# interaction-lab-uh/STROTSS-tensorflow

Measured on AMD Instinct MI355X. Metric: optimisation_steps_per_sec_1024px_pair, higher is better.
Workload: dtype f32; 1 GPU; 1024px content/style pair, 1024x1024 scale of the coarse-to-fine pyramid, 1024 samples x D=2179, VGG16 (seeded He-normal weights), RMSprop pixel update; scale_px=1024, samples=1024, parallelism=single GPU, tap_adjoint=deterministic (planned, sorted scatter)

## Files before the change

strotss-tensorflow_amd/csrc/gemm.hip:

```cpp
#include <stdlib.h>

#include "internal.h"
#include "mfma_pipe.h"
#include "mfma_x3.h"

namespace {

template <int BM, int BN, bool AKC, bool BKC>
__device__ __forceinline__ void gemm_mainloop(const float* __restrict__ A, int lda, int M,
                                              const float* __restrict__ B, int ldb, int N, int K,
                                              int m0, int n0, float* ldsA, float* ldsB,
                                              f32x16 (&acc)[BM / 64][BN / 64]) {
  f32x4 ra[BM / 32], rb[BN / 32];
  auto load = [&](int k0) {
    if constexpr (AKC) gload_kc<BM>(ra, A, lda, m0, M, k0); else gload_rc<BM>(ra, A, lda, m0, M, k0);
    if constexpr (BKC) gload_kc<BN>(rb, B, ldb, n0, N, k0); else gload_rc<BN>(rb, B, ldb, n0, N, k0);
  };
  load(0);
  for (int k0 = 0; k0 < K; k0 += 32) {
    __syncthreads();
    if constexpr (AKC) lds_store_kc<BM>(ldsA, ra); else lds_store_rc<BM>(ldsA, ra);
    if constexpr (BKC) lds_store_kc<BN>(ldsB, rb); else lds_store_rc<BN>(ldsB, rb);
    __syncthreads();
    if (k0 + 32 < K) load(k0 + 32);
// ... 340 lines not shown
  const size_t total = (size_t)rows * (K >> 2);
  hipLaunchKernelGGL(x3_split_rows_kernel, dim3((unsigned)min((size_t)2048, (total + 255) / 256), batch), dim3(256), 0, s,
                     x, rows, ld, K, stride_in, (__bf16*)panels, (long long)3 * rows * K);
  ST_LAUNCH_RET();
}

struct EpiScaleStoreX3 : EpiScaleStore, X3NoPrefetch<EpiScaleStoreX3> {
  using EpiScaleStore::apply;
  using X3NoPrefetch<EpiScaleStoreX3>::apply;
};
struct X3NoMirror {
  template <class Epi, class Pre, class Acc, class Map>
  __device__ __forceinline__ void operator()(const Epi&, Pre&, float*, int, int, int, int, Acc&, const Map&) const {}
};
template <class Cfg>
struct X3Mirror {
  template <class Epi, class Pre, class Acc, class Map>
  __device__ __forceinline__ void operator()(const Epi& epi, Pre&, float* tile, int m0, int n0, int M, int N, Acc& acc,
                                             const Map& map) const {
    mirror_tile<Cfg::BM, Cfg::BN, Cfg::NT, true>(epi, tile, m0, n0, M, N, [&](auto put) {
#pragma unroll
      for (int im = 0; im < Cfg::T; ++im)
#pragma unroll
        for (int in = 0; in < Cfg::T; ++in)
#pragma unroll
          for (int reg = 0; reg < 16; ++reg) {
            const int r = m0 + map.row(im, reg), c = n0 + map.colof(in);
            put(r, c, (r < M && c < N) ? epi.value(r, c, acc[im][in][reg]) : 0.f);
          }
    });
  }
};

int st_gemm_x3_batched(const void* A, const void* B, float* C, int ldc, long long strideC, int M, int N, int K,
                       int batch, hipStream_t s, long min_tiles128) {
  EpiScaleStoreX3 e{{C, ldc, M, N, 1.0f, strideC}, {}};
  static const bool k16 = [] { const char* v = getenv("STROTSS_X3_K16"); return !v || atoi(v) != 0; }();
  if ((long)cdiv(N, 128) * cdiv(M, 128) * batch >= min_tiles128 && k16) {
    using Cfg = X3CfgK16<3>;
    dim3 grid((unsigned)cdiv(N, 128) * cdiv(M, 128) * batch);
    hipLaunchKernelGGL((gemm_x3_kernel<Cfg, EpiScaleStoreX3, X3NoMirror>), grid, dim3(Cfg::NT), 0, s, (const __bf16*)A, M,
                       (long long)3 * M * K, (const __bf16*)B, N, (long long)3 * N * K, K, e, X3NoMirror{});
  } else if ((long)cdiv(N, 128) * cdiv(M, 128) * batch >= min_tiles128) {
    using Cfg = X3Cfg<128>;
    dim3 grid((unsigned)cdiv(N, 128) * cdiv(M, 128) * batch);
    hipLaunchKernelGGL((gemm_x3_kernel<Cfg, EpiScaleStoreX3, X3NoMirror>), grid, dim3(Cfg::NT), 0, s, (const __bf16*)A, M,
                       (long long)3 * M * K, (const __bf16*)B, N, (long long)3 * N * K, K, e, X3NoMirror{});
  } else {
    using Cfg = X3Cfg<64>;
    dim3 grid((unsigned)cdiv(N, 64) * cdiv(M, 64) * batch);
    hipLaunchKernelGGL((gemm_x3_kernel<Cfg, EpiScaleStoreX3, X3NoMirror>), grid, dim3(Cfg::NT), 0, s, (const __bf16*)A, M,
                       (long long)3 * M * K, (const __bf16*)B, N, (long long)3 * N * K, K, e, X3NoMirror{});
  }
  ST_LAUNCH_RET();
}

struct EpiSelfsimBwdX3 : EpiSelfsimBwd {
  template <int T> struct Pre { float dx0[T][T][16], x0[T][T][16], ri[T][16], qi[T][16]; };
  template <class P> __device__ __forceinline__ void prefetch(P& p, int im, int in, int reg, int row, int c) const {
    const int rr = min(row, M - 1);
    const size_t o = (size_t)rr * ld + min(c, N - 1);
    p.dx0[im][in][reg] = dx[o];
    p.x0[im][in][reg] = x[o];
    if (in == 0) { p.ri[im][reg] = r[rr]; p.qi[im][reg] = q[rr]; }
  }
  template <class P> __device__ __forceinline__ float apply(P& p, int im, int in, int reg, int row, int c, float v) const {
    const float ri = p.ri[im][reg];
    const float out = p.dx0[im][in][reg] + g * ri * (v - p.x0[im][in][reg] * ri * p.qi[im][reg]);
    if (row < M && c < N) dx[(size_t)row * ld + c] = out;
    return 0.f;
  }
};
struct EpiAxpbyBiasX3 : EpiAxpbyBias {
  template <int T> struct Pre { float c0[T][T][16], b[T]; };
  template <class P> __device__ __forceinline__ void prefetch(P& p, int im, int in, int reg, int r, int c) const {
    p.c0[im][in][reg] = C[(size_t)min(r, M - 1) * ldc + min(c, N - 1)];
    if (im == 0 && reg == 0) p.b[in] = bias[min(c, N - 1)];
  }
  template <class P> __device__ __forceinline__ float apply(P& p, int im, int in, int reg, int r, int c, float v) const {
    const float out = p.c0[im][in][reg] + alpha * v + bias_scale * p.b[in];
    if (r < M && c < N) C[(size_t)r * ldc + c] = out;
    return 0.f;
  }
};
struct EpiMomentFwdX3 {
  static constexpr bool SYMM = true;
// ... 238 lines not shown
```

strotss-tensorflow_amd/csrc/internal.h:

```cpp
#pragma once
#include "common.h"

int st_cosine_distance(const float* x, const float* rx, int nx, const float* y, const float* ry, int ny,
                       int ld, float* C, int ldc, hipStream_t s);
int st_l2_distance(const float* x, const float* xs, int nx, const float* y, const float* ys, int ny, int ld, int d,
                   float* C, int ldc, hipStream_t s);
int st_remd_cost(const float* x, const float* rx, const float* sx, int nx, const float* y, const float* ry, const float* sy,
                 int ny, int ld, int d, int metric, float* C, float* S, int ldc, hipStream_t s);
int st_gram_tn(const float* A, int krows, int ld, float alpha, float* C, hipStream_t s);
int st_moment_fwd_gemm(const float* cy, int krows, int ld, const float* Sx, float* T, float inv_n,
                       float* partial, int* n_partial, hipStream_t s);
int st_moment_bwd_gemm(const float* cy, int n, int ld, const float* T, float alpha, const float* bias,
                       float bias_scale, float* dY, hipStream_t s);
int st_selfsim_bwd_gemm(const float* Mq, int ldm, int kpad, const float* bmat, const float* x, const float* r,
                        const float* q, int n, int ld, float g, float* dx, hipStream_t s);

int st_gemm_nt_batched(const float* A, int lda, long long strideA, const float* B, int ldb, long long strideB,
                       float* C, int ldc, long long strideC, int M, int N, int K, int batch, hipStream_t s);

bool st_winograd43_fused_enabled(int h, int w, int cout);
int st_winograd43_pack(const float* u_prk, int rows, int k, float* u_packed, hipStream_t st);
int st_winograd43_fused(const float* in, int h, int w, int cin, const float* U, const float* bias, int cout,
                        const float* mask, int relu, float* out, float* pool_out, unsigned char* pool_code,
                        const unsigned* bits_in, unsigned* bits_out, hipStream_t st, int accumulate = 0);
int st_maxpool2_fwd(const float* in, int h, int w, int c, float* out, unsigned char* code, hipStream_t st);

int st_x3_split_rows(const float* x, int rows, int ld, int K, long long stride_in, void* panels, int batch,
                     hipStream_t s);
int st_cosine_distance_x3(const void* xp, const float* rx, int nx, const void* yp, const float* ry, int ny, int K,
                          int symm, float* C, int ldc, int batch, long long pstride, long long rstride,
                          long long cstride, hipStream_t s);
int st_selfsim_bwd_x3(const void* Mp, int kpad, const void* Xt, const float* x, const float* r, const float* q, int n,
                      int ld, float g, float* dx, hipStream_t s);
int st_gram_tn_x3(const void* Pt, int npad, int ld, float alpha, float* C, hipStream_t s);
int st_moment_fwd_x3(const void* Pt, int npad, int ld, const float* Sx, void* Tp, float inv_n, float* partial,
                     int* n_partial, hipStream_t s);
int st_loss_forward_group_x3(const void* Pt, int npad, int ld, const float* Sx, void* Tp, float inv_n, float* partial,
                             int* n_partial, const void* xp, const float* rp, int n, long long pstride, long long rstride,
                             float* Dx, int ldc, long long dstride, const void* xs, const float* rs, int ns, float* Ct,
                             int ldt, hipStream_t s);
int st_loss_forward_blend_x3(const void* Pt, int npad, int ld, float inv_n, float* Sigma, const void* xp, const float* rp,
                             int n, long long pstride, long long rstride, float* Dx, int ldc, long long dstride, int n_styles,
                             const void* const* xs, const float* const* rs, const int* ns, float* const* Ct, const int* ldt,
                             hipStream_t s);
int st_moment_bwd_x3_full(const void* Pc, int n, int ld, const void* Sp, float alpha, const float* bias, float bias_scale,
                          float* dY, hipStream_t s);
int st_moment_bwd_x3(const void* Pc, int n, int ld, const void* Tp, float alpha, const float* bias, float bias_scale,
                     float* dY, hipStream_t s);
int st_gemm_x3_batched(const void* A, const void* B, float* C, int ldc, long long strideC, int M, int N, int K,
                       int batch, hipStream_t s, long min_tiles128 = 0);

static inline int round_up(int v, int m) { return (v + m - 1) / m * m; }

struct Workspace {
  char* base; size_t size; size_t off;
  Workspace(void* p, size_t n) : base((char*)p), size(n), off(0) {}
  template <class T> T* take(size_t count) {
    size_t bytes = (count * sizeof(T) + 255) & ~(size_t)255;
    if (off + bytes > size) { failed = true; return nullptr; }
    T* r = reinterpret_cast<T*>(base + off);
    off += bytes;
    return r;
  }
  bool failed = false;
  bool ok() const { return !failed; }
  static Workspace planner() { return Workspace(nullptr, (size_t)1 << 60); }
};
static inline size_t ws_slice(size_t count, size_t elt) { return (count * elt + 255) & ~(size_t)255; }
```

strotss-tensorflow_amd/csrc/mfma_x3.h:

```cpp
#pragma once
#include <type_traits>

#include "mfma_pipe.h"

typedef __bf16 bf16x8 __attribute__((ext_vector_type(8)));
typedef __bf16 bf16x4 __attribute__((ext_vector_type(4)));
typedef unsigned int u32x4 __attribute__((ext_vector_type(4)));

struct Split3 { bf16x4 h, m, l; };
__device__ __forceinline__ Split3 split3(const f32x4 x) {
  Split3 s;
#pragma unroll
  for (int k = 0; k < 4; ++k) {
    const __bf16 h = (__bf16)x[k];
    const float r1 = x[k] - (float)h;
    const __bf16 m = (__bf16)r1;
    const float r2 = r1 - (float)m;
    s.h[k] = h; s.m[k] = m; s.l[k] = (__bf16)r2;
  }
  return s;
}

__host__ __device__ __forceinline__ size_t x3_panel_elems(size_t rows, size_t K) { return 3 * rows * K; }
__device__ __forceinline__ void x3_store4(__bf16* base, size_t rows, size_t row, int k0, const f32x4 v) {
  const Split3 s = split3(v);
  const size_t o = ((size_t)(k0 >> 5) * 3 * rows + row) * 32 + (k0 & 31);
  *reinterpret_cast<bf16x4*>(base + o) = s.h;
  *reinterpret_cast<bf16x4*>(base + o + rows * 32) = s.m;
  *reinterpret_cast<bf16x4*>(base + o + 2 * rows * 32) = s.l;
}

template <int B_, int NPB_ = 3>
struct X3Cfg {
  static_assert(B_ == 128 || B_ == 64, "x3 main loop: 128 x 128 or 64 x 64 tiles");
  static_assert(NPB_ == 3 || (NPB_ == 1 && B_ == 128), "single-plane B: 128 x 128 tiles only");
  static constexpr int NPB = NPB_, NPROD = NPB_ == 3 ? 6 : 3;
  static constexpr int BM = B_, BN = B_, WM = 2, WN = 2, NT = 256;
  static constexpr int T = B_ / 64;
  static constexpr int TM = T, TN = T;
  static constexpr int PL = B_ * 64;
  static constexpr int STAGE = (3 + NPB_) * PL;
  static constexpr int LDS_BYTES = 3 * STAGE;
  static constexpr int G = B_ / 64;
  static constexpr int NP = (3 + NPB_) * G;
  static constexpr bool K16 = false;
};

#define X3_WAIT_VM(n) asm volatile("s_waitcnt vmcnt(" #n ")" ::: "memory")

template <int G, int NPL = 3>
struct X3Operand {
  const char* base;
  unsigned off[G];
  unsigned plane;
  unsigned cur;
  __device__ __forceinline__ X3Operand(const __bf16* p, int rows, int row0) {
    const int lane = threadIdx.x & 63, wave = __builtin_amdgcn_readfirstlane(threadIdx.x >> 6);
    base = reinterpret_cast<const char*>(p);
    plane = (unsigned)rows * 64u;
    cur = 0;
    const int chunk = (lane & 3) ^ ((lane >> 4) & 3);
#pragma unroll
    for (int g = 0; g < G; ++g) {
      const int row = min(row0 + (G * wave + g) * 16 + (lane >> 2), rows - 1);
      off[g] = (unsigned)row * 64u + (unsigned)chunk * 16u;
    }
  }
  __device__ __forceinline__ void dma(int pl, int g, unsigned char* lds_dst) const {
    const char* src = base + (size_t)(cur + pl * plane) + off[g];
    __builtin_amdgcn_global_load_lds((const __attribute__((address_space(1))) void*)src,
                                     (__attribute__((address_space(3))) void*)lds_dst, 16, 0, 0);
  }
  __device__ __forceinline__ void advance() { cur += NPL * plane; }
};

template <class Cfg>
__device__ __forceinline__ void x3_mainloop(unsigned char* lds, int steps, X3Operand<Cfg::G, 3>& oa,
                                            X3Operand<Cfg::G, Cfg::NPB>& ob, f32x16 (&acc)[Cfg::T][Cfg::T]) {
// ... 69 lines not shown
#else
            acc[im][in_][0] += (float)fa[c][PA[q]][im][0] + (float)fb[c][PB[q]][in_][0];
#endif
            const int done = (q * T + im) * T + in_ + 1;
            if (MODE == 2 && c == 0 && done % STRIDE == 0 && done / STRIDE <= NP) {
              __builtin_amdgcn_sched_barrier(0);
              dma_piece(done / STRIDE - 1, s_nn);
              __builtin_amdgcn_sched_barrier(0);
            }
          }
        }
        if (c == 1 && q == 0 && MODE != 0) {
          __builtin_amdgcn_sched_barrier(0);
          if (MODE == 2) wait_one_tile_in_flight(); else X3_WAIT_VM(0);
          asm volatile("s_waitcnt lgkmcnt(0)" ::: "memory");
#ifndef X3_ABL_NO_BARRIER
          __builtin_amdgcn_s_barrier();
#endif
          asm volatile("" ::: "memory");
          read_frags(s_nxt, 0, 0);
          __builtin_amdgcn_sched_barrier(0);
        }
      }
    }
    if (MODE == 2) { oa.advance(); ob.advance(); }
    unsigned char* tmp = s_cur; s_cur = s_nxt; s_nxt = s_nn; s_nn = tmp;
  };
  int s = 0;
  for (; s + 2 < steps; ++s) kstep(std::integral_constant<int, 2>{});
  if (steps > 1) kstep(std::integral_constant<int, 1>{});
  kstep(std::integral_constant<int, 0>{});
}

template <int NPB_ = 3>
struct X3CfgK16 {
  static_assert(NPB_ == 3, "K16 ring: three B planes");
  static constexpr int NPB = NPB_, NPROD = 6;
  static constexpr int BM = 128, BN = 128, WM = 2, WN = 2, NT = 256;
  static constexpr int T = 2, TM = 2, TN = 2;
  static constexpr int PL = 128 * 32;
  static constexpr int STAGE = 6 * PL;
  static constexpr int LDS_BYTES = 3 * STAGE;
  static constexpr int G = 1, NP = 6;
  static constexpr bool K16 = true;
};

struct X3OperandK16 {
  const char* base;
  unsigned off;
  unsigned plane;
  unsigned cur;
  __device__ __forceinline__ X3OperandK16(const __bf16* p, int rows, int row0) {
    const int lane = threadIdx.x & 63, wave = __builtin_amdgcn_readfirstlane(threadIdx.x >> 6);
    base = reinterpret_cast<const char*>(p);
    plane = (unsigned)rows * 64u;
    cur = 0;
    const int row = min(row0 + wave * 32 + (lane >> 1), rows - 1);
    off = (unsigned)row * 64u + (unsigned)((lane & 1) ^ ((lane >> 4) & 1)) * 16u;
  }
  __device__ __forceinline__ void dma(int pl, unsigned char* lds_dst) const {
    const char* src = base + (size_t)(cur + pl * plane) + off;
    __builtin_amdgcn_global_load_lds((const __attribute__((address_space(1))) void*)src,
                                     (__attribute__((address_space(3))) void*)lds_dst, 16, 0, 0);
  }
  __device__ __forceinline__ void advance(int half) { cur += half ? 3u * plane - 32u : 32u; }
};

template <class Cfg> struct X3Ops {
  using A = std::conditional_t<Cfg::K16, X3OperandK16, X3Operand<Cfg::G, 3>>;
  using B = std::conditional_t<Cfg::K16, X3OperandK16, X3Operand<Cfg::G, Cfg::NPB>>;
};

template <class Cfg>
__device__ __forceinline__ void x3_k16_prologue(unsigned char* lds, X3OperandK16& oa, X3OperandK16& ob) {
#ifndef X3_ABL_NO_DMA
  const int wave = __builtin_amdgcn_readfirstlane(threadIdx.x >> 6);
#pragma unroll
  for (int h = 0; h < 2; ++h) {
    unsigned char* stage = lds + h * Cfg::STAGE;
#pragma unroll
    for (int j = 0; j < 6; ++j) {
      unsigned char* dst = stage + j * Cfg::PL + wave * 1024;
      if (j < 3) oa.dma(j, dst); else ob.dma(j - 3, dst);
    }
    oa.advance(h); ob.advance(h);
  }
#endif
}

template <class Cfg>
__device__ __forceinline__ void x3_mainloop_k16(unsigned char* lds, int steps, X3OperandK16& oa, X3OperandK16& ob,
                                                f32x16 (&acc)[2][2]) {
  constexpr int PL = Cfg::PL, STAGE = Cfg::STAGE;
  const int t = threadIdx.x, lane = t & 63, wave = __builtin_amdgcn_readfirstlane(t >> 6);
  const int wm = wave >> 1, wn = wave & 1, l31 = lane & 31, hh = lane >> 5;
  auto dma_piece = [&](int j, unsigned char* stage) {
#ifdef X3_ABL_NO_DMA
    return;
#endif
    unsigned char* dst = stage + j * PL + wave * 1024;
    if (j < 3) oa.dma(j, dst); else ob.dma(j - 3, dst);
  };
  int half = 0;
  const int sw = (hh ^ ((l31 >> 3) & 1)) << 4;
  const int a_rd = (wm * 64 + l31) * 32 + sw;
  const int b_rd = 3 * PL + (wn * 64 + l31) * 32 + sw;
  bf16x8 fa[2][3][2], fb[2][3][2];
  auto read_frags = [&](const unsigned char* stage, int slot) {
#ifdef X3_ABL_NO_FRAG
    if (stage != lds) return;
#endif
#pragma unroll
    for (int p = 0; p < 3; ++p) {
#pragma unroll
      for (int i = 0; i < 2; ++i) {
        fa[slot][p][i] = *reinterpret_cast<const bf16x8*>(stage + a_rd + p * PL + i * 1024);
        fb[slot][p][i] = *reinterpret_cast<const bf16x8*>(stage + b_rd + p * PL + i * 1024);
      }
    }
  };
  constexpr int PA[6] = {2, 0, 1, 1, 0, 0};
  constexpr int PB[6] = {0, 2, 1, 0, 1, 0};

  unsigned char* s_cur = lds;
  unsigned char* s_nxt = lds + STAGE;
  unsigned char* s_nn = lds + 2 * STAGE;
  X3_WAIT_VM(6);
  __builtin_amdgcn_s_barrier();
  read_frags(s_cur, 0);

  auto kstep = [&](auto mode_tag, auto slot_tag) {
    constexpr int MODE = decltype(mode_tag)::value, SLOT = decltype(slot_tag)::value;
#pragma unroll
    for (int q = 0; q < 6; ++q) {
#pragma unroll
      for (int im = 0; im < 2; ++im) {
#pragma unroll
        for (int in_ = 0; in_ < 2; ++in_) {
#ifndef X3_ABL_NO_MFMA
          acc[im][in_] = __builtin_amdgcn_mfma_f32_32x32x16_bf16(fa[SLOT][PA[q]][im], fb[SLOT][PB[q]][in_], acc[im][in_], 0, 0, 0);
#else
          acc[im][in_][0] += (float)fa[SLOT][PA[q]][im][0] + (float)fb[SLOT][PB[q]][in_][0];
#endif
          const int done = (q * 2 + im) * 2 + in_ + 1;
          if (MODE == 2 && done <= 6) {
            __builtin_amdgcn_sched_barrier(0);
            dma_piece(done - 1, s_nn);
            __builtin_amdgcn_sched_barrier(0);
          }
        }
      }
      if (q == 3 && MODE != 0) {
        __builtin_amdgcn_sched_barrier(0);
        if (MODE == 2) X3_WAIT_VM(6); else X3_WAIT_VM(0);
        asm volatile("s_waitcnt lgkmcnt(0)" ::: "memory");
#ifndef X3_ABL_NO_BARRIER
        __builtin_amdgcn_s_barrier();
#endif
        asm volatile("" ::: "memory");
        read_frags(s_nxt, SLOT ^ 1);
        __builtin_amdgcn_sched_barrier(0);
      }
    }
    if (MODE == 2) { oa.advance(half); ob.advance(half); half ^= 1; }
    unsigned char* tmp = s_cur; s_cur = s_nxt; s_nxt = s_nn; s_nn = tmp;
  };
  using I0 = std::integral_constant<int, 0>; using I1 = std::integral_constant<int, 1>; using I2 = std::integral_constant<int, 2>;
  int s = 0;
  for (; s + 3 < steps; s += 2) { kstep(I2{}, I0{}); kstep(I2{}, I1{}); }
  kstep(I1{}, I0{});
  kstep(I0{}, I1{});
}

template <class D>
struct X3NoPrefetch {
  template <int T> struct Pre {};
  template <class P> __device__ __forceinline__ void prefetch(P&, int, int, int, int, int) const {}
  template <class P> __device__ __forceinline__ float apply(P&, int, int, int, int r, int c, float v) const {
    return static_cast<const D*>(this)->apply(r, c, v);
  }
};

template <class Cfg, class Epi, class Mirror>
__device__ __forceinline__ void gemm_x3_tile(unsigned char* lds, unsigned bid, unsigned nblk, const __bf16* __restrict__ A, int M,
                                             long long strideA, const __bf16* __restrict__ B, int N, long long strideB, int K,
                                             const Epi& epi_in, const Mirror& mirror, int xbh, int xbw) {
  Epi epi = epi_in;
  const unsigned gx = (N + Cfg::BN - 1) / Cfg::BN, gy = (M + Cfg::BM - 1) / Cfg::BM;
  unsigned tile = xcd_swizzle(bid, nblk);
  unsigned bz = 0;
  int m0, n0;
  bool tri = false;
  if constexpr (Epi::SYMM) tri = epi.symm != 0;
  if (tri) {
    const unsigned ntri = gx * (gx + 1) / 2;
    bz = tile / ntri;
    tile -= bz * ntri;
    unsigned i = 0, len = gx;
    while (tile >= len) { tile -= len; --len; ++i; }
    m0 = i * Cfg::BM; n0 = (i + tile) * Cfg::BN;
  } else {
    bz = tile / (gx * gy);
    const unsigned rem = tile - bz * (gx * gy);
    if (xbh > 0) {
      const unsigned per = (unsigned)(xbh * xbw), blk = rem / per, in = rem - blk * per;
      const unsigned bpr = gx / (unsigned)xbw;
      const unsigned ty = (blk / bpr) * xbh + in / xbw, tx = (blk % bpr) * xbw + in % xbw;
      m0 = ty * Cfg::BM; n0 = tx * Cfg::BN;
    } else {
      m0 = (rem / gx) * Cfg::BM; n0 = (rem % gx) * Cfg::BN;
    }
  }
  epi.set_batch(bz);
  typename X3Ops<Cfg>::A oa(A + (long long)bz * strideA, M, m0);
  typename X3Ops<Cfg>::B ob(B + (long long)bz * strideB, N, n0);
  f32x16 acc[Cfg::T][Cfg::T];
#pragma unroll
  for (int i = 0; i < Cfg::T; ++i)
#pragma unroll
    for (int j = 0; j < Cfg::T; ++j)
#pragma unroll
      for (int r = 0; r < 16; ++r) acc[i][j][r] = 0.f;
  PipeAccMap<Cfg> map;
  typename Epi::template Pre<Cfg::T> pre;
#pragma unroll
  for (int im = 0; im < Cfg::T; ++im)
#pragma unroll
    for (int in = 0; in < Cfg::T; ++in)
#pragma unroll
      for (int reg = 0; reg < 16; ++reg)
        epi.prefetch(pre, im, in, reg, m0 + map.row(im, reg), n0 + map.colof(in));
  if constexpr (Cfg::K16) { x3_k16_prologue<Cfg>(lds, oa, ob); x3_mainloop_k16<Cfg>(lds, K >> 4, oa, ob, acc); }
  else x3_mainloop<Cfg>(lds, K >> 5, oa, ob, acc);
  float local = 0.f;
#pragma unroll
  for (int im = 0; im < Cfg::T; ++im)
#pragma unroll
    for (int in = 0; in < Cfg::T; ++in)
#pragma unroll
      for (int reg = 0; reg < 16; ++reg)
        local += epi.apply(pre, im, in, reg, m0 + map.row(im, reg), n0 + map.colof(in), acc[im][in][reg]);
  if constexpr (Epi::SYMM) {
    static_assert(!Epi::SYMM || Cfg::LDS_BYTES >= Cfg::BM * (Cfg::BN + 1) * 4, "mirror tile");
    if (epi.symm && n0 >= m0) mirror(epi, pre, reinterpret_cast<float*>(lds), m0, n0, M, N, acc, map);
  }
  __syncthreads();
  epi.finish(reinterpret_cast<float*>(lds), local);
}

template <class Cfg, class Epi, class Mirror>
__global__ __launch_bounds__(Cfg::NT) void gemm_x3_kernel(const __bf16* __restrict__ A, int M, long long strideA,
                                                          const __bf16* __restrict__ B, int N, long long strideB,
                                                          int K, Epi epi, Mirror mirror, int xbh = 0, int xbw = 0) {
  __shared__ __attribute__((aligned(1024))) unsigned char lds[Cfg::LDS_BYTES];
  gemm_x3_tile<Cfg, Epi, Mirror>(lds, blockIdx.x, gridDim.x, A, M, strideA, B, N, strideB, K, epi, mirror, xbh, xbw);
}

template <class Epi>
struct X3Problem {
  const __bf16* A; int M; long long strideA;
  const __bf16* B; int N; long long strideB;
  int K; Epi epi; int xbh, xbw;
  unsigned n;
};
__host__ __device__ __forceinline__ unsigned x3_pad8(unsigned n) { return (n + 7u) & ~7u; }
template <class C0, class E0, class M0, class C1, class E1, class M1, class C2, class E2, class M2>
__global__ __launch_bounds__(256) void gemm_x3_group3_kernel(X3Problem<E0> p0, X3Problem<E1> p1, X3Problem<E2> p2) {
  static_assert(C0::NT == 256 && C1::NT == 256 && C2::NT == 256, "grouped x3 launch: 256-thread workgroups");
  constexpr int L01 = C0::LDS_BYTES > C1::LDS_BYTES ? C0::LDS_BYTES : C1::LDS_BYTES;
  constexpr int LDSB = L01 > C2::LDS_BYTES ? L01 : C2::LDS_BYTES;
  __shared__ __attribute__((aligned(1024))) unsigned char lds[LDSB];
  unsigned b = blockIdx.x;
  if (b < x3_pad8(p0.n)) {
    if (b < p0.n) { M0 m; gemm_x3_tile<C0, E0, M0>(lds, b, p0.n, p0.A, p0.M, p0.strideA, p0.B, p0.N, p0.strideB, p0.K, p0.epi, m, p0.xbh, p0.xbw); }
    return;
  }
  b -= x3_pad8(p0.n);
  if (b < x3_pad8(p1.n)) {
    if (b < p1.n) { M1 m; gemm_x3_tile<C1, E1, M1>(lds, b, p1.n, p1.A, p1.M, p1.strideA, p1.B, p1.N, p1.strideB, p1.K, p1.epi, m, p1.xbh, p1.xbw); }
    return;
  }
  b -= x3_pad8(p1.n);
  if (b < p2.n) { M2 m; gemm_x3_tile<C2, E2, M2>(lds, b, p2.n, p2.A, p2.M, p2.strideA, p2.B, p2.N, p2.strideB, p2.K, p2.epi, m, p2.xbh, p2.xbw); }
}
// ... 47 lines not shown
```

strotss-tensorflow_amd/csrc/winograd.hip:

```cpp
#include <stdlib.h>

#include "internal.h"
#include "mfma_x3.h"

namespace {

__global__ __launch_bounds__(256) void winograd_in_kernel(const float* __restrict__ in, int H, int W, int C4,
                                                          int TH, int TW, size_t tile0, size_t T,
                                                          float* __restrict__ V) {
  const size_t total = T * C4;
  const f32x4* src = reinterpret_cast<const f32x4*>(in);
  f32x4* dst = reinterpret_cast<f32x4*>(V);
  auto put = [&](int pos, size_t tile, int c, const f32x4 v) { dst[((size_t)pos * T + tile) * C4 + c] = v; };
  for (size_t e = (size_t)blockIdx.x * 256 + threadIdx.x; e < total; e += (size_t)gridDim.x * 256) {
    const int c = (int)(e % C4);
    const size_t tile = e / C4;
    const size_t gt = tile0 + tile;
    const int tx = (int)(gt % TW), ty = (int)(gt / TW);
    f32x4 d[4][4];
#pragma unroll
    for (int r = 0; r < 4; ++r) {
      const int y = 2 * ty - 1 + r;
#pragma unroll
      for (int q = 0; q < 4; ++q) {
// ... 97 lines not shown
  f32x4* dst = reinterpret_cast<f32x4*>(V);
  for (unsigned e = blockIdx.x * 256u + threadIdx.x; e < total; e += gridDim.x * 256u) {
    unsigned tile; int c;
    split_index(e, C4, c4_shift, tile, c);
    const int ty = (int)(tile / (unsigned)TW), tx = (int)(tile - (unsigned)ty * (unsigned)TW);
    f32x4 d[6][6];
#pragma unroll
    for (int r = 0; r < 6; ++r) {
      const int y = 4 * ty - 1 + r;
#pragma unroll
      for (int q = 0; q < 6; ++q) {
        const int x = 4 * tx - 1 + q;
        f32x4 v = {0.f, 0.f, 0.f, 0.f};
        if (y >= 0 && y < H && x >= 0 && x < W) v = src[((size_t)y * W + x) * C4 + c];
        d[r][q] = v;
      }
    }
#pragma unroll
    for (int q = 0; q < 6; ++q) {
      f32x4 col[6] = {d[0][q], d[1][q], d[2][q], d[3][q], d[4][q], d[5][q]};
      bt6(col);
#pragma unroll
      for (int r = 0; r < 6; ++r) d[r][q] = col[r];
    }
#pragma unroll
    for (int r = 0; r < 6; ++r) {
      bt6(d[r]);
#pragma unroll
      for (int q = 0; q < 6; ++q) dst[((size_t)(r * 6 + q) * T + tile) * C4 + c] = d[r][q];
    }
  }
}

__global__ __launch_bounds__(256) void winograd43_in_x3_kernel(const float* __restrict__ in, int H, int W, int C4,
                                                               int TH, int TW, __bf16* __restrict__ V, int kb_shift) {
  const size_t T = (size_t)TH * TW;
  const int KB = C4 >> 3;
  const unsigned total = (unsigned)(((T + 7) >> 3) * 64 * KB);
  const f32x4* src = reinterpret_cast<const f32x4*>(in);
  const size_t panel = 3 * T * (size_t)C4 * 4;
  for (unsigned e = blockIdx.x * 256u + threadIdx.x; e < total; e += gridDim.x * 256u) {
    const int c8 = (int)(e & 7), tlo = (int)((e >> 3) & 7);
    unsigned r8; int kb;
    split_index(e >> 6, KB, kb_shift, r8, kb);
    const unsigned tile = r8 * 8 + tlo;
    if (tile >= T) continue;
    const int c = kb * 8 + c8;
    const int ty = (int)(tile / (unsigned)TW), tx = (int)(tile - (unsigned)ty * (unsigned)TW);
    f32x4 d[6][6];
#pragma unroll
    for (int rr = 0; rr < 6; ++rr) {
      const int y = 4 * ty - 1 + rr;
#pragma unroll
      for (int q = 0; q < 6; ++q) {
        const int x = 4 * tx - 1 + q;
        f32x4 v = {0.f, 0.f, 0.f, 0.f};
        if (y >= 0 && y < H && x >= 0 && x < W) v = src[((size_t)y * W + x) * C4 + c];
        d[rr][q] = v;
      }
    }
#pragma unroll
    for (int q = 0; q < 6; ++q) {
      f32x4 col[6] = {d[0][q], d[1][q], d[2][q], d[3][q], d[4][q], d[5][q]};
      bt6(col);
#pragma unroll
      for (int rr = 0; rr < 6; ++rr) d[rr][q] = col[rr];
    }
#pragma unroll
    for (int rr = 0; rr < 6; ++rr) {
      bt6(d[rr]);
#pragma unroll
      for (int q = 0; q < 6; ++q) x3_store4(V + (size_t)(rr * 6 + q) * panel, T, tile, 4 * c, d[rr][q]);
    }
  }
}

__global__ __launch_bounds__(256) void winograd43_out_kernel(const float* __restrict__ Mw, int H, int W, int C4,
                                                             int TH, int TW, const float* __restrict__ bias,
                                                             const float* __restrict__ mask, int relu,
                                                             float* __restrict__ out, int c4_shift, size_t Tstride,
                                                             const u32x4* __restrict__ bits_in, u32x4* __restrict__ bits_out,
                                                             f32x4* __restrict__ pool, unsigned* __restrict__ pool_code,
                                                             int accumulate) {
  const size_t T = (size_t)TH * TW;
  const unsigned total = (unsigned)(T * C4);
  const f32x4* src = reinterpret_cast<const f32x4*>(Mw);
  const f32x4* msk = reinterpret_cast<const f32x4*>(mask);
  f32x4* dst = reinterpret_cast<f32x4*>(out);
  for (unsigned e = blockIdx.x * 256u + threadIdx.x; e < total; e += gridDim.x * 256u) {
    unsigned tile; int c;
    split_index(e, C4, c4_shift, tile, c);
    const int ty = (int)(tile / (unsigned)TW), tx = (int)(tile - (unsigned)ty * (unsigned)TW);
    f32x4 s[4][6];
#pragma unroll
    for (int q = 0; q < 6; ++q) {
      f32x4 m[6];
#pragma unroll
      for (int r = 0; r < 6; ++r) m[r] = src[((size_t)(r * 6 + q) * Tstride + tile) * C4 + c];
      s[0][q] = m[0] + m[1] + m[2] + m[3] + m[4];
      s[1][q] = m[1] - m[2] + 2.f * m[3] - 2.f * m[4];
      s[2][q] = m[1] + m[2] + 4.f * m[3] + 4.f * m[4];
      s[3][q] = m[1] - m[2] + 8.f * m[3] - 8.f * m[4] + m[5];
    }
    f32x4 b = {0.f, 0.f, 0.f, 0.f};
    if (bias) b = reinterpret_cast<const f32x4*>(bias)[c];
    u32x4 kw = {0u, 0u, 0u, 0u}, ow = {0u, 0u, 0u, 0u};
    if (bits_in) kw = bits_in[e];
// ... 44 lines not shown
            for (int j = 0; j < 4; ++j) {
              const float v4[4] = {prev[2 * pc][j], prev[2 * pc + 1][j], yv[2 * pc][j], yv[2 * pc + 1][j]};
              int best = 0;
              float bv = v4[0];
#pragma unroll
              for (int k = 1; k < 4; ++k)
                if (v4[k] > bv) { bv = v4[k]; best = k; }
              pv[j] = fmaxf(bv, 0.f);
              packed |= (unsigned)(bv > 0.f ? best : 4) << (8 * j);
            }
            const size_t po = ((size_t)py * PW + px) * C4 + c;
            pool[po] = pv;
            if (pool_code) pool_code[po] = packed;
          }
        }
      }
    }
    if (bits_out) bits_out[e] = ow;
  }
}

static long x3_min_tiles() {
  static long min_tiles = -1;
  if (min_tiles < 0) { const char* m = getenv("STROTSS_X3_MIN_TILES"); min_tiles = m ? atol(m) : 1024; }
  return min_tiles;
}
static bool x3_enabled(size_t T, int cout) {
  static int on = -1;
  if (on < 0) {
    const char* c = getenv("STROTSS_X3_CONV"); on = c ? atoi(c) : 1;
    const char* e = getenv("STROTSS_X3"); if (e && atoi(e) == 0) on = 0;
  }
  return on != 0 && (long)((T + 63) / 64) * ((cout + 63) / 64) * 36 >= x3_min_tiles();
}

static int x3_min_cout() {
  static int v = -1;
  if (v < 0) { const char* e = getenv("STROTSS_X3_MIN_COUT"); v = e ? atoi(e) : 256; }
  return v;
}
static bool winograd43_prefers_x3(int h, int w, int cout) {
  const size_t T = (size_t)((h + 3) / 4) * ((w + 3) / 4);
  return cout >= x3_min_cout() && x3_enabled(T, cout) && (long)((T + 127) / 128) * ((cout + 127) / 128) * 36 >= x3_min_tiles();
}

static int g_wino_stages = 7;

static int winograd43_run(const float* in, int h, int w, int cin, const float* U, const float* Upacked,
                          const void* Ux3, const float* bias, int cout, const float* mask, int relu, float* out,
                          float* pool_out, unsigned char* pool_code, void* workspace, size_t workspace_bytes,
                          hipStream_t st, const unsigned* bits_in = nullptr, unsigned* bits_out = nullptr, int accumulate = 0) {
  const bool prefer_x3 = Ux3 && cin % 32 == 0 && winograd43_prefers_x3(h, w, cout);
  if (!prefer_x3 && Upacked && cin % 32 == 0 && st_winograd43_fused_enabled(h, w, cout))
    return st_winograd43_fused(in, h, w, cin, Upacked, bias, cout, mask, relu, out, pool_out, pool_code, bits_in, bits_out, st,
                               accumulate);
  const int TH = (h + 3) / 4, TW = (w + 3) / 4;
  const size_t T = (size_t)TH * TW;
  const bool x3 = Ux3 && cin % 32 == 0 && x3_enabled(T, cout);
  if (T * (size_t)(max(cin, cout) / 4 + 8) >= (1ull << 32)) return STROTSS_ERANGE;
  Workspace ws(workspace, workspace_bytes);
  float* V = ws.take<float>(36 * T * cin * 3 / 2);
  float* Mw = ws.take<float>(36 * T * cout);
  if (!ws.ok()) return STROTSS_EINVAL;
  const size_t tout = T * (cout / 4);
  const size_t Tstride = T;
  int rc;
  const int stages = g_wino_stages;
  if (x3) {
    const size_t tin = ((T + 7) / 8) * 8 * (cin / 4);
    if (stages & 1) hipLaunchKernelGGL(winograd43_in_x3_kernel, dim3((unsigned)min((size_t)16384, (tin + 255) / 256)), dim3(256), 0, st,
                       in, h, w, cin / 4, TH, TW, reinterpret_cast<__bf16*>(V), log2_or_minus1(cin / 32));
    if (!(stages & 2)) rc = 0;
    else rc = st_gemm_x3_batched(V, Ux3, Mw, cout, (long long)T * cout, (int)T, cout, cin, 36, st, x3_min_tiles());
  } else {
    const size_t tin = T * (cin / 4);
    if (stages & 1) hipLaunchKernelGGL(winograd43_in_kernel, dim3((unsigned)min((size_t)16384, (tin + 255) / 256)), dim3(256), 0, st, in,
                       h, w, cin / 4, TH, TW, V, log2_or_minus1(cin / 4));
    rc = (stages & 2) ? st_gemm_nt_batched(V, cin, (long long)T * cin, U, cin, (long long)cout * cin, Mw, cout,
                                           (long long)T * cout, (int)T, cout, cin, 36, st) : 0;
  }
  if (rc != 0) return rc;
  static const bool out_pools = [] { const char* v = getenv("STROTSS_WINO_OUT_POOL"); return !v || atoi(v) != 0; }();
  if (stages & 4) hipLaunchKernelGGL(winograd43_out_kernel, dim3((unsigned)min((size_t)16384, (tout + 255) / 256)), dim3(256), 0, st,
                     Mw, h, w, cout / 4, TH, TW, bias, mask, relu, out, log2_or_minus1(cout / 4), Tstride,
                     reinterpret_cast<const u32x4*>(bits_in), reinterpret_cast<u32x4*>(bits_out),
                     reinterpret_cast<f32x4*>(out_pools ? pool_out : nullptr),
                     reinterpret_cast<unsigned*>(out_pools ? pool_code : nullptr), accumulate);
  if (pool_out && !out_pools) return st_maxpool2_fwd(out, h, w, cout, pool_out, pool_code, st);
  ST_LAUNCH_RET();
}

static size_t wino_chunk_tiles(size_t T, int cin, int cout) {
  static long mb = -1;
  if (mb < 0) { const char* e = getenv("STROTSS_WINO_CHUNK_MB"); mb = e ? atol(e) : 0; }
  if (mb == 0) return T;
  size_t tc = ((size_t)mb << 20) / ((size_t)16 * (cin + cout) * sizeof(float));
  tc = tc / 128 * 128;
  if (tc < 1024) tc = 1024;
  return tc < T ? tc : T;
}

int winograd_run(const float* in, int h, int w, int cin, const float* U, const float* bias, int cout,
                 const float* mask, int relu, float* out, void* workspace, size_t workspace_bytes,
                 hipStream_t st) {
  const int TH = (h + 1) / 2, TW = (w + 1) / 2;
  const size_t T = (size_t)TH * TW;
// ... 144 lines not shown
```

Before: 222.7 steps/s.

## Feed fp32 Winograd input to x3 GEMM and split to bf16 in-kernel

The Winograd input transform now writes fp32 K-blocked panels instead of three bf16 split planes. A new K16 GEMM variant DMAs those fp32 tiles into LDS and does the hi/mid/lo bf16 split in registers after reading the fragments. This cuts the transform's write traffic and the GEMM's A-operand read traffic from 3×bf16 to 1×fp32 per element, and shrinks the A part of each LDS stage from three planes to two. In exchange the GEMM inner loop does extra split arithmetic, and the wait point moves earlier in the product sequence (WQ=1) to suit the five in-flight DMA pieces, which could expose latency.

```diff
diff --git a/strotss-tensorflow_amd/csrc/gemm.hip b/strotss-tensorflow_amd/csrc/gemm.hip
--- a/strotss-tensorflow_amd/csrc/gemm.hip
+++ b/strotss-tensorflow_amd/csrc/gemm.hip
@@ -396,11 +396,14 @@
   }
 };
 
+static bool x3_k16_enabled() {
+  static const bool k16 = [] { const char* v = getenv("STROTSS_X3_K16"); return !v || atoi(v) != 0; }();
+  return k16;
+}
 int st_gemm_x3_batched(const void* A, const void* B, float* C, int ldc, long long strideC, int M, int N, int K,
                        int batch, hipStream_t s, long min_tiles128) {
   EpiScaleStoreX3 e{{C, ldc, M, N, 1.0f, strideC}, {}};
-  static const bool k16 = [] { const char* v = getenv("STROTSS_X3_K16"); return !v || atoi(v) != 0; }();
-  if ((long)cdiv(N, 128) * cdiv(M, 128) * batch >= min_tiles128 && k16) {
+  if ((long)cdiv(N, 128) * cdiv(M, 128) * batch >= min_tiles128 && x3_k16_enabled()) {
     using Cfg = X3CfgK16<3>;
     dim3 grid((unsigned)cdiv(N, 128) * cdiv(M, 128) * batch);
     hipLaunchKernelGGL((gemm_x3_kernel<Cfg, EpiScaleStoreX3, X3NoMirror>), grid, dim3(Cfg::NT), 0, s, (const __bf16*)A, M,
@@ -416,6 +419,20 @@
     hipLaunchKernelGGL((gemm_x3_kernel<Cfg, EpiScaleStoreX3, X3NoMirror>), grid, dim3(Cfg::NT), 0, s, (const __bf16*)A, M,
                        (long long)3 * M * K, (const __bf16*)B, N, (long long)3 * N * K, K, e, X3NoMirror{});
   }
+  ST_LAUNCH_RET();
+}
+
+bool st_gemm_x3_f32a_ok(int M, int N, int batch, long min_tiles128) {
+  return (long)cdiv(N, 128) * cdiv(M, 128) * batch >= min_tiles128 && x3_k16_enabled();
+}
+int st_gemm_x3_batched_f32a(const float* A, const void* B, float* C, int ldc, long long strideC, int M, int N, int K,
+                            int batch, hipStream_t s, long min_tiles128) {
+  if (!st_gemm_x3_f32a_ok(M, N, batch, min_tiles128)) return STROTSS_EINVAL;
+  EpiScaleStoreX3 e{{C, ldc, M, N, 1.0f, strideC}, {}};
+  using Cfg = X3CfgK16<3, true>;
+  dim3 grid((unsigned)cdiv(N, 128) * cdiv(M, 128) * batch);
+  hipLaunchKernelGGL((gemm_x3_kernel<Cfg, EpiScaleStoreX3, X3NoMirror>), grid, dim3(Cfg::NT), 0, s, A, M, (long long)M * K,
+                     (const __bf16*)B, N, (long long)3 * N * K, K, e, X3NoMirror{});
   ST_LAUNCH_RET();
 }
 
diff --git a/strotss-tensorflow_amd/csrc/internal.h b/strotss-tensorflow_amd/csrc/internal.h
--- a/strotss-tensorflow_amd/csrc/internal.h
+++ b/strotss-tensorflow_amd/csrc/internal.h
@@ -49,6 +49,9 @@
                      float* dY, hipStream_t s);
 int st_gemm_x3_batched(const void* A, const void* B, float* C, int ldc, long long strideC, int M, int N, int K,
                        int batch, hipStream_t s, long min_tiles128 = 0);
+bool st_gemm_x3_f32a_ok(int M, int N, int batch, long min_tiles128);
+int st_gemm_x3_batched_f32a(const float* A, const void* B, float* C, int ldc, long long strideC, int M, int N, int K,
+                            int batch, hipStream_t s, long min_tiles128);
 
 static inline int round_up(int v, int m) { return (v + m - 1) / m * m; }
 
diff --git a/strotss-tensorflow_amd/csrc/mfma_x3.h b/strotss-tensorflow_amd/csrc/mfma_x3.h
--- a/strotss-tensorflow_amd/csrc/mfma_x3.h
+++ b/strotss-tensorflow_amd/csrc/mfma_x3.h
@@ -43,7 +43,7 @@
   static constexpr int LDS_BYTES = 3 * STAGE;
   static constexpr int G = B_ / 64;
   static constexpr int NP = (3 + NPB_) * G;
-  static constexpr bool K16 = false;
+  static constexpr bool K16 = false, AF32 = false;
 };
 
 #define X3_WAIT_VM(n) asm volatile("s_waitcnt vmcnt(" #n ")" ::: "memory")
@@ -179,16 +179,21 @@
   kstep(std::integral_constant<int, 0>{});
 }
 
-template <int NPB_ = 3>
+template <int NPB_ = 3, bool AF32_ = false, int WQ_ = AF32_ ? 1 : 3>
 struct X3CfgK16 {
   static_assert(NPB_ == 3, "K16 ring: three B planes");
+  static_assert(WQ_ >= 0 && WQ_ <= 4, "K16 ring: the wait needs at least one product group after it");
   static constexpr int NPB = NPB_, NPROD = 6;
+  static constexpr bool AF32 = AF32_;
+  static constexpr int WQ = WQ_;
   static constexpr int BM = 128, BN = 128, WM = 2, WN = 2, NT = 256;
   static constexpr int T = 2, TM = 2, TN = 2;
   static constexpr int PL = 128 * 32;
-  static constexpr int STAGE = 6 * PL;
+  static constexpr int NPA = AF32_ ? 2 : 3;
+  static constexpr int ABYTES = NPA * PL;
+  static constexpr int STAGE = ABYTES + 3 * PL;
   static constexpr int LDS_BYTES = 3 * STAGE;
-  static constexpr int G = 1, NP = 6;
+  static constexpr int G = 1, NP = NPA + 3;
   static constexpr bool K16 = true;
 };
 
@@ -213,57 +218,115 @@
   __device__ __forceinline__ void advance(int half) { cur += half ? 3u * plane - 32u : 32u; }
 };
 
+struct X3OperandK16F32 {
+  const char* base;
+  unsigned off[2];
+  unsigned kblk;
+  unsigned cur;
+  __device__ __forceinline__ X3OperandK16F32(const float* p, int rows, int row0) {
+    const int lane = threadIdx.x & 63, wave = __builtin_amdgcn_readfirstlane(threadIdx.x >> 6);
+    base = reinterpret_cast<const char*>(p);
+    kblk = (unsigned)rows * 128u;
+    cur = 0;
+    const int chunk = (lane & 3) ^ ((lane >> 4) & 3);
+#pragma unroll
+    for (int g = 0; g < 2; ++g) {
+      const int row = min(row0 + wave * 32 + g * 16 + (lane >> 2), rows - 1);
+      off[g] = (unsigned)row * 128u + (unsigned)chunk * 16u;
+    }
+  }
+  __device__ __forceinline__ void dma(int g, unsigned char* lds_dst) const {
+    const char* src = base + (size_t)cur + off[g];
+    __builtin_amdgcn_global_load_lds((const __attribute__((address_space(1))) void*)src,
+                                     (__attribute__((address_space(3))) void*)lds_dst, 16, 0, 0);
+  }
+  __device__ __forceinline__ void advance(int half) { cur += half ? kblk - 64u : 64u; }
+};
+
+__device__ __forceinline__ void x3_f32_store4(float* base, size_t rows, size_t row, int k0, const f32x4 v) {
+  *reinterpret_cast<f32x4*>(base + ((size_t)(k0 >> 5) * rows + row) * 32 + (k0 & 31)) = v;
+}
+
+__device__ __forceinline__ void x3_split8(const f32x4 lo, const f32x4 hi, bf16x8& h, bf16x8& m, bf16x8& l) {
+  const Split3 a = split3(lo), b = split3(hi);
+  h = __builtin_shufflevector(a.h, b.h, 0, 1, 2, 3, 4, 5, 6, 7);
+  m = __builtin_shufflevector(a.m, b.m, 0, 1, 2, 3, 4, 5, 6, 7);
+  l = __builtin_shufflevector(a.l, b.l, 0, 1, 2, 3, 4, 5, 6, 7);
+}
+
 template <class Cfg> struct X3Ops {
-  using A = std::conditional_t<Cfg::K16, X3OperandK16, X3Operand<Cfg::G, 3>>;
+  using A = std::conditional_t<Cfg::K16, std::conditional_t<Cfg::AF32, X3OperandK16F32, X3OperandK16>, X3Operand<Cfg::G, 3>>;
   using B = std::conditional_t<Cfg::K16, X3OperandK16, X3Operand<Cfg::G, Cfg::NPB>>;
-};
-
-template <class Cfg>
-__device__ __forceinline__ void x3_k16_prologue(unsigned char* lds, X3OperandK16& oa, X3OperandK16& ob) {
+  using AT = std::conditional_t<Cfg::AF32, float, __bf16>;
+};
+
+template <class Cfg, class OA>
+__device__ __forceinline__ void x3_k16_prologue(unsigned char* lds, OA& oa, X3OperandK16& ob) {
 #ifndef X3_ABL_NO_DMA
   const int wave = __builtin_amdgcn_readfirstlane(threadIdx.x >> 6);
 #pragma unroll
   for (int h = 0; h < 2; ++h) {
     unsigned char* stage = lds + h * Cfg::STAGE;
 #pragma unroll
-    for (int j = 0; j < 6; ++j) {
-      unsigned char* dst = stage + j * Cfg::PL + wave * 1024;
-      if (j < 3) oa.dma(j, dst); else ob.dma(j - 3, dst);
+    for (int j = 0; j < Cfg::NP; ++j) {
+      if (j >= Cfg::NPA) ob.dma(j - Cfg::NPA, stage + Cfg::ABYTES + (j - Cfg::NPA) * Cfg::PL + wave * 1024);
+      else if constexpr (Cfg::AF32) oa.dma(j, stage + wave * 2048 + j * 1024);
+      else oa.dma(j, stage + j * Cfg::PL + wave * 1024);
     }
     oa.advance(h); ob.advance(h);
   }
 #endif
 }
 
-template <class Cfg>
-__device__ __forceinline__ void x3_mainloop_k16(unsigned char* lds, int steps, X3OperandK16& oa, X3OperandK16& ob,
+template <class Cfg, class OA>
+__device__ __forceinline__ void x3_mainloop_k16(unsigned char* lds, int steps, OA& oa, X3OperandK16& ob,
                                                 f32x16 (&acc)[2][2]) {
-  constexpr int PL = Cfg::PL, STAGE = Cfg::STAGE;
+  constexpr int PL = Cfg::PL, STAGE = Cfg::STAGE, NPA = Cfg::NPA, NP = Cfg::NP, WQ = Cfg::WQ;
+  constexpr bool AF32 = Cfg::AF32;
+  static_assert(NP == 5 || NP == 6, "K16 ring: 5 or 6 DMA pieces per wave and step");
   const int t = threadIdx.x, lane = t & 63, wave = __builtin_amdgcn_readfirstlane(t >> 6);
   const int wm = wave >> 1, wn = wave & 1, l31 = lane & 31, hh = lane >> 5;
   auto dma_piece = [&](int j, unsigned char* stage) {
 #ifdef X3_ABL_NO_DMA
     return;
 #endif
-    unsigned char* dst = stage + j * PL + wave * 1024;
-    if (j < 3) oa.dma(j, dst); else ob.dma(j - 3, dst);
+    if (j >= NPA) ob.dma(j - NPA, stage + Cfg::ABYTES + (j - NPA) * PL + wave * 1024);
+    else if constexpr (AF32) oa.dma(j, stage + wave * 2048 + j * 1024);
+    else oa.dma(j, stage + j * PL + wave * 1024);
+  };
+  constexpr int IN_FLIGHT = 4 * (WQ + 1) < NP ? 4 * (WQ + 1) : NP;
+  auto wait_next_tile = [&]() {
+    if constexpr (IN_FLIGHT == 6) X3_WAIT_VM(6); else if constexpr (IN_FLIGHT == 5) X3_WAIT_VM(5); else X3_WAIT_VM(4);
   };
   int half = 0;
   const int sw = (hh ^ ((l31 >> 3) & 1)) << 4;
   const int a_rd = (wm * 64 + l31) * 32 + sw;
-  const int b_rd = 3 * PL + (wn * 64 + l31) * 32 + sw;
+  const int b_rd = Cfg::ABYTES + (wn * 64 + l31) * 32 + sw;
+  const int af = (l31 >> 2) & 3;
+  const int a_rd0 = (wm * 64 + l31) * 64 + (((2 * hh) ^ af) << 4), a_rd1 = (wm * 64 + l31) * 64 + (((2 * hh + 1) ^ af) << 4);
   bf16x8 fa[2][3][2], fb[2][3][2];
+  f32x4 ra[2][2];
   auto read_frags = [&](const unsigned char* stage, int slot) {
 #ifdef X3_ABL_NO_FRAG
     if (stage != lds) return;
 #endif
 #pragma unroll
-    for (int p = 0; p < 3; ++p) {
-#pragma unroll
-      for (int i = 0; i < 2; ++i) {
-        fa[slot][p][i] = *reinterpret_cast<const bf16x8*>(stage + a_rd + p * PL + i * 1024);
+    for (int i = 0; i < 2; ++i) {
+      if constexpr (AF32) {
+        ra[i][0] = *reinterpret_cast<const f32x4*>(stage + a_rd0 + i * 2048);
+        ra[i][1] = *reinterpret_cast<const f32x4*>(stage + a_rd1 + i * 2048);
+      }
+#pragma unroll
+      for (int p = 0; p < 3; ++p) {
+        if constexpr (!AF32) fa[slot][p][i] = *reinterpret_cast<const bf16x8*>(stage + a_rd + p * PL + i * 1024);
         fb[slot][p][i] = *reinterpret_cast<const bf16x8*>(stage + b_rd + p * PL + i * 1024);
       }
+    }
+  };
+  auto split_a = [&](int slot) {
+    if constexpr (AF32) {
+#pragma unroll
+      for (int i = 0; i < 2; ++i) x3_split8(ra[i][0], ra[i][1], fa[slot][0][i], fa[slot][1][i], fa[slot][2][i]);
     }
   };
   constexpr int PA[6] = {2, 0, 1, 1, 0, 0};
@@ -272,9 +335,10 @@
   unsigned char* s_cur = lds;
   unsigned char* s_nxt = lds + STAGE;
   unsigned char* s_nn = lds + 2 * STAGE;
-  X3_WAIT_VM(6);
+  if constexpr (NP == 6) X3_WAIT_VM(6); else X3_WAIT_VM(5);
   __builtin_amdgcn_s_barrier();
   read_frags(s_cur, 0);
+  split_a(0);
 
   auto kstep = [&](auto mode_tag, auto slot_tag) {
     constexpr int MODE = decltype(mode_tag)::value, SLOT = decltype(slot_tag)::value;
@@ -290,16 +354,16 @@
           acc[im][in_][0] += (float)fa[SLOT][PA[q]][im][0] + (float)fb[SLOT][PB[q]][in_][0];
 #endif
           const int done = (q * 2 + im) * 2 + in_ + 1;
-          if (MODE == 2 && done <= 6) {
+          if (MODE == 2 && done <= NP) {
             __builtin_amdgcn_sched_barrier(0);
             dma_piece(done - 1, s_nn);
             __builtin_amdgcn_sched_barrier(0);
           }
         }
       }
-      if (q == 3 && MODE != 0) {
+      if (q == WQ && MODE != 0) {
         __builtin_amdgcn_sched_barrier(0);
-        if (MODE == 2) X3_WAIT_VM(6); else X3_WAIT_VM(0);
+        if (MODE == 2) wait_next_tile(); else X3_WAIT_VM(0);
         asm volatile("s_waitcnt lgkmcnt(0)" ::: "memory");
 #ifndef X3_ABL_NO_BARRIER
         __builtin_amdgcn_s_barrier();
@@ -307,6 +371,7 @@
         asm volatile("" ::: "memory");
         read_frags(s_nxt, SLOT ^ 1);
         __builtin_amdgcn_sched_barrier(0);
+        split_a(SLOT ^ 1);
       }
     }
     if (MODE == 2) { oa.advance(half); ob.advance(half); half ^= 1; }
@@ -329,7 +394,8 @@
 };
 
 template <class Cfg, class Epi, class Mirror>
-__device__ __forceinline__ void gemm_x3_tile(unsigned char* lds, unsigned bid, unsigned nblk, const __bf16* __restrict__ A, int M,
+__device__ __forceinline__ void gemm_x3_tile(unsigned char* lds, unsigned bid, unsigned nblk,
+                                             const typename X3Ops<Cfg>::AT* __restrict__ A, int M,
                                              long long strideA, const __bf16* __restrict__ B, int N, long long strideB, int K,
                                              const Epi& epi_in, const Mirror& mirror, int xbh, int xbw) {
   Epi epi = epi_in;
@@ -396,7 +462,7 @@
 }
 
 template <class Cfg, class Epi, class Mirror>
-__global__ __launch_bounds__(Cfg::NT) void gemm_x3_kernel(const __bf16* __restrict__ A, int M, long long strideA,
+__global__ __launch_bounds__(Cfg::NT) void gemm_x3_kernel(const typename X3Ops<Cfg>::AT* __restrict__ A, int M, long long strideA,
                                                           const __bf16* __restrict__ B, int N, long long strideB,
                                                           int K, Epi epi, Mirror mirror, int xbh = 0, int xbw = 0) {
   __shared__ __attribute__((aligned(1024))) unsigned char lds[Cfg::LDS_BYTES];
diff --git a/strotss-tensorflow_amd/csrc/winograd.hip b/strotss-tensorflow_amd/csrc/winograd.hip
--- a/strotss-tensorflow_amd/csrc/winograd.hip
+++ b/strotss-tensorflow_amd/csrc/winograd.hip
@@ -153,13 +153,13 @@
   }
 }
 
-__global__ __launch_bounds__(256) void winograd43_in_x3_kernel(const float* __restrict__ in, int H, int W, int C4,
-                                                               int TH, int TW, __bf16* __restrict__ V, int kb_shift) {
+template <class Store>
+__device__ __forceinline__ void winograd43_in_k_blocked(const float* __restrict__ in, int H, int W, int C4, int TH, int TW,
+                                                        int kb_shift, const Store& store) {
   const size_t T = (size_t)TH * TW;
   const int KB = C4 >> 3;
   const unsigned total = (unsigned)(((T + 7) >> 3) * 64 * KB);
   const f32x4* src = reinterpret_cast<const f32x4*>(in);
-  const size_t panel = 3 * T * (size_t)C4 * 4;
   for (unsigned e = blockIdx.x * 256u + threadIdx.x; e < total; e += gridDim.x * 256u) {
     const int c8 = (int)(e & 7), tlo = (int)((e >> 3) & 7);
     unsigned r8; int kb;
@@ -191,9 +191,25 @@
     for (int rr = 0; rr < 6; ++rr) {
       bt6(d[rr]);
 #pragma unroll
-      for (int q = 0; q < 6; ++q) x3_store4(V + (size_t)(rr * 6 + q) * panel, T, tile, 4 * c, d[rr][q]);
-    }
-  }
+      for (int q = 0; q < 6; ++q) store(rr * 6 + q, tile, 4 * c, d[rr][q]);
+    }
+  }
+}
+
+__global__ __launch_bounds__(256) void winograd43_in_x3_kernel(const float* __restrict__ in, int H, int W, int C4,
+                                                               int TH, int TW, __bf16* __restrict__ V, int kb_shift) {
+  const size_t T = (size_t)TH * TW, panel = 3 * T * (size_t)C4 * 4;
+  winograd43_in_k_blocked(in, H, W, C4, TH, TW, kb_shift, [&](int p, unsigned tile, int k0, const f32x4 v) {
+    x3_store4(V + (size_t)p * panel, T, tile, k0, v);
+  });
+}
+
+__global__ __launch_bounds__(256) void winograd43_in_f32k_kernel(const float* __restrict__ in, int H, int W, int C4,
+                                                                 int TH, int TW, float* __restrict__ V, int kb_shift) {
+  const size_t T = (size_t)TH * TW, panel = T * (size_t)C4 * 4;
+  winograd43_in_k_blocked(in, H, W, C4, TH, TW, kb_shift, [&](int p, unsigned tile, int k0, const f32x4 v) {
+    x3_f32_store4(V + (size_t)p * panel, T, tile, k0, v);
+  });
 }
 
 __global__ __launch_bounds__(256) void winograd43_out_kernel(const float* __restrict__ Mw, int H, int W, int C4,
@@ -304,6 +320,12 @@
     const char* e = getenv("STROTSS_X3"); if (e && atoi(e) == 0) on = 0;
   }
   return on != 0 && (long)((T + 63) / 64) * ((cout + 63) / 64) * 36 >= x3_min_tiles();
+}
+
+static bool x3_f32a_enabled() {
+  static int on = -1;
+  if (on < 0) { const char* e = getenv("STROTSS_X3_CONV_F32A"); on = e ? atoi(e) : 1; }
+  return on != 0;
 }
 
 static int x3_min_cout() {
@@ -340,10 +362,16 @@
   const int stages = g_wino_stages;
   if (x3) {
     const size_t tin = ((T + 7) / 8) * 8 * (cin / 4);
-    if (stages & 1) hipLaunchKernelGGL(winograd43_in_x3_kernel, dim3((unsigned)min((size_t)16384, (tin + 255) / 256)), dim3(256), 0, st,
-                       in, h, w, cin / 4, TH, TW, reinterpret_cast<__bf16*>(V), log2_or_minus1(cin / 32));
-    if (!(stages & 2)) rc = 0;
-    else rc = st_gemm_x3_batched(V, Ux3, Mw, cout, (long long)T * cout, (int)T, cout, cin, 36, st, x3_min_tiles());
+    const dim3 gin((unsigned)min((size_t)16384, (tin + 255) / 256));
+    if (x3_f32a_enabled() && st_gemm_x3_f32a_ok((int)T, cout, 36, x3_min_tiles())) {
+      if (stages & 1) hipLaunchKernelGGL(winograd43_in_f32k_kernel, gin, dim3(256), 0, st, in, h, w, cin / 4, TH, TW, V,
+                                         log2_or_minus1(cin / 32));
+      rc = (stages & 2) ? st_gemm_x3_batched_f32a(V, Ux3, Mw, cout, (long long)T * cout, (int)T, cout, cin, 36, st, x3_min_tiles()) : 0;
+    } else {
+      if (stages & 1) hipLaunchKernelGGL(winograd43_in_x3_kernel, gin, dim3(256), 0, st, in, h, w, cin / 4, TH, TW,
+                                         reinterpret_cast<__bf16*>(V), log2_or_minus1(cin / 32));
+      rc = (stages & 2) ? st_gemm_x3_batched(V, Ux3, Mw, cout, (long long)T * cout, (int)T, cout, cin, 36, st, x3_min_tiles()) : 0;
+    }
   } else {
     const size_t tin = T * (cin / 4);
     if (stages & 1) hipLaunchKernelGGL(winograd43_in_kernel, dim3((unsigned)min((size_t)16384, (tin + 255) / 256)), dim3(256), 0, st, in,
```

Result: faster. 226.1 steps/s, median of 6 (+1.5%).
